# ouc-ocean-group/RRNet

Hardware: AMD Instinct MI355X
Metric: images/sec (train step) (higher is better)
Workload: dtype f32; 1 GPU; RRNet hourglass-104 (2 stacks) train step, 1024x1024 synthetic VisDrone frames, fp32; per_gpu_batch=8, global_batch=8, k=1500, parallelism=dp1

## Files before the change

rrnet_amd/_C.py:

```python
import ctypes
import os

import torch

_HERE = os.path.dirname(os.path.abspath(__file__))
LIB_PATH = os.path.join(_HERE, "librrnet_hip.so")
_lib = None

c_int, c_float, c_void_p, c_size_t = ctypes.c_int, ctypes.c_float, ctypes.c_void_p, ctypes.c_size_t
c_long, c_double = ctypes.c_long, ctypes.c_double


class RRNetHipError(RuntimeError):
    pass


def lib():
    global _lib
    if _lib is None:
        global LIB_PATH
        LIB_PATH = os.environ.get("RRNET_HIP_LIB", LIB_PATH)
        if not os.path.exists(LIB_PATH):
            raise RRNetHipError(
                "librrnet_hip.so not found at %s — build it with `python rrnet_amd/csrc/build.py` "
# ... 51 lines not shown
                    argtypes.append(_CTYPE[toks[0]])
                    pointees.append("hipStream_t" if toks[0] == "hipStream_t" else None)
        sigs[name] = Signature((restype, argtypes))
        sigs[name].pointees = tuple(pointees)
    return sigs


def header_signatures():
    global _SIGS
    if _SIGS is None:
        _SIGS = _parse_header(MAIN_HEADER)
    return _SIGS


MAIN_HEADER = "rrnet_hip.h"
COMPANION_HEADERS = ("rrnet_hip_se.h", "rrnet_hip_attn.h", "rrnet_hip_dw.h", "rrnet_hip_rows.h")
_FAMILY_SIGS = {}


def family_signatures(header):
    if header not in COMPANION_HEADERS:
        raise RRNetHipError("%s is not a header of this library (%s)" % (header, ", ".join((MAIN_HEADER,) + COMPANION_HEADERS)))
    if header not in _FAMILY_SIGS:
        _FAMILY_SIGS[header] = _parse_header(header)
    return _FAMILY_SIGS[header]


def declared(name):
    sig = header_signatures().get(name)
    if sig is not None:
        return sig, MAIN_HEADER
# ... 93 lines not shown
```

rrnet_amd/csrc/build.py:

```python
import os
import subprocess
import sys
from concurrent.futures import ThreadPoolExecutor

HERE = os.path.dirname(os.path.abspath(__file__))
ROOT = os.path.dirname(os.path.dirname(HERE))
INC = os.path.join(ROOT, "include")
OUT = os.path.join(os.path.dirname(HERE), "librrnet_hip.so")
HIPCC = os.environ.get("HIPCC", "/opt/rocm/bin/hipcc")
COMMON = ["--offload-arch=gfx950", "-O3", "-fPIC", "-std=c++17", "-I", INC, "-I", HERE,
          "-Wno-unused-result", "-fno-gpu-rdc"]
PER_FILE = {
    "softnms.hip": ["-ffp-contract=off"],
    "hardnms.hip": ["-ffp-contract=off"],
    "refine.hip": ["-ffp-contract=off"],
    "targets.hip": ["-ffp-contract=off"],
    "psroi.hip": ["-ffp-contract=off"],
    "augment.hip": ["-ffp-contract=off"],
    "augment_paste.hip": ["-ffp-contract=off"],
    "jitter.hip": ["-ffp-contract=off"],
    "evalmatch.hip": ["-ffp-contract=off"],
    "detect.hip": ["-ffp-contract=off"],
    "retina.hip": ["-ffp-contract=off"],
    "kmeans.hip": ["-ffp-contract=off"],
    "wbf.hip": ["-ffp-contract=off"],
    "textio.hip": ["-ffp-contract=off"],
    "depthwise.hip": ["-ffp-contract=off"],
}


def sources():
    return sorted(f for f in os.listdir(HERE) if f.endswith(".hip") or f.endswith(".cpp"))


def _stale(obj, src):
    if not os.path.exists(obj):
        return True
    t = os.path.getmtime(obj)
    deps = [os.path.join(HERE, src)] + [os.path.join(INC, h) for h in os.listdir(INC) if h.endswith(".h")] + \
           [os.path.join(HERE, h) for h in os.listdir(HERE) if h.endswith(".h")]
    return any(os.path.getmtime(d) > t for d in deps)

# ... 31 lines not shown
```

rrnet_amd/csrc/conv.hip:

```cpp
#include "conv_launch.h"
#include <hip/amd_detail/amd_hip_unsafe_atomics.h>

namespace {

typedef float f32x4 __attribute__((ext_vector_type(4)));
typedef float f32x16 __attribute__((ext_vector_type(16)));

__device__ float rr_zero16[4] = {0.f, 0.f, 0.f, 0.f};

constexpr int BM = 128;
constexpr int BK = 32;

struct ConvArgs {
    const float *src;
    const float *w;
    float *dst;
    const float *bias;
    double *stat_slab;
    const float *bs_y, *bs_z, *bs_mean, *bs_invstd, *bs_msc, *bs_msh;
    int bs_relu_bias;
    int N;
    int SH, SW, SC;
    int DH, DW, DC;
    int R, S, stride, pad_h, pad_w;
    int relu, accumulate;
    int M;
    int Kg;
    int wK, wC;
    const float *zero;
    int ksplit;
    int parity_order;
    int parity;
    int dst32;
    int pos_major;
    const int *gate;
    int gate_max;
};

__device__ __forceinline__ int xcd_remap(int bid, int nb)
{
    const int q = nb >> 3, r = nb & 7, xcd = bid & 7, idx = bid >> 3;
    return (xcd < r ? xcd * (q + 1) : r * (q + 1) + (xcd - r) * q) + idx;
}

template <int BN, int MODE, bool SCALAR, int BKT, int PIPE, bool BNS = false, bool POSM = false>
__global__ __launch_bounds__(256, PIPE == 2 ? 3 : 1) void conv_igemm_kernel(const ConvArgs a)
{
    static_assert(BKT == 32 && (PIPE == 0 || PIPE == 2), "conv_igemm_kernel: K-step 32, PIPE 0 or 2");
    if constexpr (MODE == 0 && !BNS && !POSM) {
        if (a.gate != nullptr && *a.gate <= a.gate_max) return;
    }
    constexpr int WN = BN / 64 ? BN / 64 : 1;
    constexpr int WM = 4 / WN;
    constexpr int TM = BM / (WM * 32);
    constexpr int TN = BN / (WN * 32);
    constexpr bool B_KN = (MODE == 1);
    constexpr int LDK = BKT + 4;
    constexpr int LDB = B_KN ? BN : LDK;
    constexpr int A_ELEMS = BM * LDK;
    constexpr int B_ELEMS = B_KN ? BKT * BN : BN * LDK;
    constexpr int CPR = BKT / 4;
    constexpr int RPP = 256 / CPR;
    constexpr int AJ = BM / RPP;
// ... 313 lines not shown
    auto sub = [&](const f32x4 (&fa)[TM], const f32x4 (&fb)[TN], int e) {
#pragma unroll
        for (int i = 0; i < TM; ++i)
#pragma unroll
            for (int j = 0; j < TN; ++j)
                acc[i][j] = __builtin_amdgcn_mfma_f32_32x32x2f32(fa[i][e], fb[j][e], acc[i][j], 0, 0, 0);
        __builtin_amdgcn_sched_barrier(0);
    };
    auto make_srd = [](const float *p, long bytes) {
        const unsigned long long u = reinterpret_cast<unsigned long long>(p);
        const unsigned lo = __builtin_amdgcn_readfirstlane((unsigned)u);
        const unsigned hi = __builtin_amdgcn_readfirstlane((unsigned)(u >> 32));
        void *q = reinterpret_cast<void *>(((unsigned long long)hi << 32) | lo);
        return __builtin_amdgcn_make_buffer_rsrc(q, 0, __builtin_amdgcn_readfirstlane((int)bytes), 0x00020000);
    };
    const __amdgpu_buffer_rsrc_t rs_src = make_srd(a.src, (long)a.N * a.SH * a.SW * a.SC * 4);
    const __amdgpu_buffer_rsrc_t rs_w = make_srd(a.w, (long)a.wK * RS * a.wC * 4);
    constexpr unsigned OOB = 0xFFFFFFF0u;
    int a_boff[AJ], b_boff[BJ];
#pragma unroll
    for (int j = 0; j < AJ; ++j) a_boff[j] = (int)(a_base[j] * 4);
#pragma unroll
    for (int j = 0; j < BJ; ++j) b_boff[j] = (int)(b_base[j] * 4);
    int p_cch = kc_lo / RSc, p_tl = kc_lo - (kc_lo / RSc) * RSc;
    int p_ri = p_tl / Sc, p_si = p_tl - (p_tl / Sc) * Sc;
    int p_adelta = 0, p_wdelta = 0, p_c0 = 0, p_tlc = 0;
    bool p_cok = false, p_wcok = false, p_live = true;
    auto prep = [&]() {
        const int tap = (r0 + tstep * p_ri) * a.S + (s0 + tstep * p_si);
        p_c0 = p_cch * BKT;
        p_tlc = p_tl;
        p_adelta = (sgn * (p_ri * a.SW + p_si) * a.SC + p_c0) * 4;
// ... 66 lines not shown
    }
    }

    double *sred = reinterpret_cast<double *>(lds);
    const bool do_stats = (MODE == 0) && a.stat_slab != nullptr && a.ksplit <= 1;
    constexpr bool bnsum = BNS;
    auto bs_srd = [](const float *p, long bytes) {
        const unsigned long long u = reinterpret_cast<unsigned long long>(p);
        const unsigned lo = __builtin_amdgcn_readfirstlane((unsigned)u);
        const unsigned hi = __builtin_amdgcn_readfirstlane((unsigned)(u >> 32));
        void *q = reinterpret_cast<void *>(((unsigned long long)hi << 32) | lo);
        return __builtin_amdgcn_make_buffer_rsrc(q, 0, __builtin_amdgcn_readfirstlane((int)bytes), 0x00020000);
    };
    const __amdgpu_buffer_rsrc_t bs_rs_y = bs_srd(BNS ? a.bs_y : a.src, (long)a.M * a.DC * 4);
    const __amdgpu_buffer_rsrc_t bs_rs_z = bs_srd(BNS && a.bs_z != nullptr ? a.bs_z : a.src, (long)a.M * a.DC * 4);
    const __amdgpu_buffer_rsrc_t rs_dst = bs_srd(a.dst, a.dst32 ? (long)a.M * a.DC * 4 : 0);
    constexpr unsigned OOBD = 0xFFFFFFF0u;
    const int mode_e = a.ksplit > 1 ? 2 : (a.accumulate ? 1 : 0);
    auto put_stats = [&](int j, float s1, float s2) {
        double d1 = (double)s1, d2 = (double)s2;
        d1 += __shfl_xor(d1, 32, 64);
        d2 += __shfl_xor(d2, 32, 64);
        if (lh == 0) {
            const int cl = (wn * TN + j) * 32 + lr;
            sred[(wm * BN + cl) * 2 + 0] = d1;
            sred[(wm * BN + cl) * 2 + 1] = d2;
        }
    };
    auto put_tile = [&](const f32x16 &c, const unsigned (&off)[16], float bv, float &s1, float &s2, int mode)
                        __attribute__((always_inline)) {
        const bool relu = MODE == 0 && a.relu;
// ... 620 lines not shown
    }
    if (bn == 64)
        return small ? IG(64, false, 2) : IG(64, false, 0);
    return scalar ? IG(32, true, 0) : IG(32, false, 0);
#undef IG
}

}

extern "C" size_t rr_conv_stat_slab_bytes(int n, int p, int q, int k)
{
    const long M = (long)n * p * q;
    return (size_t)((M + BM - 1) / BM) * 2 * k * sizeof(double);
}

int rr_conv_colstats(const float *y, long M, int C, double *slab, hipStream_t stream, const char *name)
{
    const int lanes = 256 / (C / 4);
    int sblocks = rr_cdiv(M, (long)lanes * 8);
    if (sblocks > 256) sblocks = 256;
    hipLaunchKernelGGL(colstats_kernel, dim3(sblocks), dim3(256), 0, stream, y, M, C, slab);
    RR_CHECK_LAUNCH(name);
    return RR_OK;
}

static int fprop_impl(const char *name, const float *x, const float *w, const float *bias, float *y, double *stat_slab,
                      int n, int h, int wd, int c, int k, int r, int s, int stride, int pad_h,
                      int pad_w, int relu, int accumulate, hipStream_t stream, const BnSumArgs *bs = nullptr, const int *gate = nullptr,
                      int gate_max = 0)
{
// ... 293 lines not shown
```

rrnet_amd/csrc/conv_launch.h:

```cpp
#pragma once
#include "common.h"
#include "conv_plan.h"
#include "rrnet_hip.h"
#include "rrnet_hip_rows.h"

struct BnSumArgs {
    const float *y, *z, *mean, *invstd, *msc, *msh;
    double *slab;
    double *sums;
    int relu_bias;
    bool bn_ok(int c) const { return y && mean && invstd && slab && sums && (!msc == !msh) && c % 4 == 0 && c <= 1024; }
    bool relu_bias_ok(int c, int k) const { return z && slab && sums && c % 4 == 0 && k % 4 == 0 && c <= 1024; }
    template <typename A> void into(A &a) const
    {
        a.stat_slab = slab; a.bs_y = y; a.bs_z = z; a.bs_mean = mean; a.bs_invstd = invstd; a.bs_msc = msc; a.bs_msh = msh; a.bs_relu_bias = relu_bias;
    }
};

template <typename K, typename A>
inline int rr_launch(K kern, dim3 grid, int threads, size_t lds, hipStream_t stream, const A &args, const char *name)
{
    if (lds > 48 * 1024)
        RR_CHECK_HIP(hipFuncSetAttribute(reinterpret_cast<const void *>(kern), hipFuncAttributeMaxDynamicSharedMemorySize, (int)lds), name);
    hipLaunchKernelGGL(kern, grid, dim3(threads), lds, stream, args);
    RR_CHECK_LAUNCH(name);
    return RR_OK;
}

inline int rr_refuse(const char *name, const rr_plan::Refusal &r)
{
    char why[256];
    snprintf(why, sizeof(why), r.why, r.a[0], r.a[1], r.a[2], r.a[3], r.a[4]);
    rr_set_error("%s: %s", name, why);
    return RR_ERR_ARG;
}

inline int rr_conv_link(const BnSumArgs *bs) { return bs == nullptr ? rr_plan::LINK_NONE : (bs->relu_bias ? rr_plan::LINK_RELU_BIAS : rr_plan::LINK_BN); }

int rr_conv_colstats(const float *y, long M, int C, double *slab, hipStream_t stream, const char *name);

int rr_gated_zero(float *p, size_t bytes, const int *count, int max_rows, int when_rows, hipStream_t stream, const char *name);

inline int rr_conv_before_launch(const rr_plan::FpropPlan &pl, int n, int k, float *y, double *stat_slab, hipStream_t stream, const char *name)
{
    RR_CHECK_HIP(rr_zero2(pl.zero_dst ? y : nullptr, pl.zero_dst ? sizeof(float) * (size_t)pl.M * k : 0, pl.zero_slab ? stat_slab : nullptr,
                          pl.zero_slab ? rr_conv_stat_slab_bytes(n, pl.dh, pl.dw, k) : 0, stream), name);
    return RR_OK;
}

inline int rr_conv_after_launch(const rr_plan::FpropPlan &pl, const BnSumArgs *bs, int k, const float *y, double *stat_slab, hipStream_t stream,
                                const char *name)
{
    switch (pl.after) {
    case rr_plan::AFTER_REDUCE_SLAB: return rr_bn_reduce_slab(bs->slab, rr_cdiv(pl.M, rr_plan::BM), k, bs->sums, stream);
// ... 64 lines not shown
```

rrnet_amd/csrc/conv_plan.h:

```cpp
#pragma once
#include <stdlib.h>

namespace rr_plan {

enum { MATH_F32 = 0, MATH_BF16 = 1, MATH_F16X3 = 2 };
enum { FAM_CONV16 = 3 };
enum { LINK_NONE = 0, LINK_BN = 1, LINK_RELU_BIAS = 2 };
enum { AFTER_NONE = 0, AFTER_REDUCE_SLAB = 1, AFTER_BWD_REDUCE = 2, AFTER_COLSTATS = 3 };

constexpr int BM = 128;
constexpr int BK = 32;

inline int cdiv(long a, long b) { return (int)((a + b - 1) / b); }

inline int mid_tiles() { return 48; }
inline int small_tiles() { return 16; }

inline int pick_ksplit(int blocks, int nk)
{
    static int enabled = -1;
    if (enabled < 0) {
        const char *e = getenv("RR_CONV_SPLITK");
        enabled = (e && atoi(e) == 0) ? 0 : 1;
    }
// ... 306 lines not shown

inline RowsPlan rows_plan(int max_rows, int c, int k, int r, int s)
{
    RowsPlan p{};
    p.dgrad_x = cdiv(max_rows, ROWS_DGRAD_BM);
    p.dgrad_y = cdiv(c, 128);
    p.mt = cdiv(k, 128); p.nt = cdiv(c, 128);
    const int tiles = p.mt * p.nt * r * s;
    p.splits = ROWS_WGRAD_SLOTS / tiles > 1 ? ROWS_WGRAD_SLOTS / tiles : 1;
    const int most = cdiv(cdiv(max_rows, BK), ROWS_WGRAD_MIN_CHUNKS);
    if (p.splits > most) p.splits = most;
    p.wgrad_grid = tiles * p.splits;
    return p;
}

}
```

rrnet_amd/flat.py:

```python
import os

import torch
import torch.distributed as dist

from rrnet_amd import dptrace, ops


class FlatParams:

    def __init__(self, module, bucket_elems=16 * 1024 * 1024):
        params = [p for p in module.parameters() if p.requires_grad]
        assert params, "no trainable parameters"
        dev = params[0].device
        offs, total = [], 0
        for p in params:
            offs.append(total)
            total += (p.numel() + 3) // 4 * 4
        self.flat = torch.zeros(total, dtype=torch.float32, device=dev)
        self.grad = torch.zeros(total, dtype=torch.float32, device=dev)
        self.params = params
        self.numel = total
        for p, o in zip(params, offs):
            n = p.numel()
            if p.dim() == 4:
# ... 17 lines not shown
            if end - start >= bucket_elems or i + 1 == len(params):
                self._bucket_range.append((start, end))
                self._bucket_need.append(need)
                start, need = end, 0
        self._index_of = {id(p): i for i, p in enumerate(params)}
        self._offs = {id(p): o for p, o in zip(params, offs)}
        self._names = {id(p): name for name, p in module.named_parameters()}
        self.wt_flat = None
        self.w16_flat = self.wt16_flat = None
        self._wt_table = None
        self._wt_tabled = set()
        self.epoch = 0
        self._wt_version = None
        self._wt_pver = {}
        self._wt_enabled = True and dev.type == "cuda"
        self.overlap = os.environ.get("RR_DP_OVERLAP", "1") != "0"
        self._pg = None
        self._begin_step()

    def _build_wt_table(self):
        import numpy as np
        rows = []
        self._wt_tabled = set()
        for p in self.params:
            if p.dim() != 4:
                continue
            k, c, r, s = p.shape
            if k > 65535 or r * s >= 2048 or (k + 31) // 32 > 1023 or (c + 31) // 32 > 1023:
                continue
            self._wt_tabled.add(id(p))
            o = self._offs[id(p)]
            kt, ct = (k + 31) // 32, (c + 31) // 32
            tap, ki, ci = np.meshgrid(np.arange(r * s), np.arange(kt), np.arange(ct), indexing="ij")
            n = tap.size
            t = np.empty((n, 4), dtype=np.int32)
            t[:, 0] = o
            t[:, 1] = ((r * s) << 16) | k
            t[:, 2] = c
            t[:, 3] = (tap.reshape(-1) << 20) | (ki.reshape(-1) << 10) | ci.reshape(-1)
            rows.append(t)
        tab = np.concatenate(rows) if rows else np.zeros((0, 4), dtype=np.int32)
        self._wt_table = torch.from_numpy(tab).to(self.flat.device)

    def refresh_wt(self):
        if not self._wt_enabled or self.wt_flat is None:
            return
        from rrnet_amd import _C
        if self.w16_flat is not None:
            _C.call("rr_weight_flip_transpose_batch_bf16", self.flat, self.wt_flat, self.w16_flat, self.wt16_flat, self._wt_table,
                    self._wt_table.shape[0])
        else:
            _C.call("rr_weight_flip_transpose_batch", self.flat, self.wt_flat, self._wt_table, self._wt_table.shape[0])
        self._wt_version = self.flat._version
        self._wt_pver = {id(p): p._version for p in self.params if p.dim() == 4}

    def invalidate_wt(self):
        self._wt_version = None
        self.epoch += 1

    def _wt_ready(self, p, bf16):
        if not self._wt_enabled or p.dim() != 4 or id(p) not in self._offs:
            return False
        if self.wt_flat is None:
            self._build_wt_table()
            self.wt_flat = torch.empty_like(self.flat)
            self._wt_version = None
        if bf16 and self.w16_flat is None:
            self.w16_flat = torch.empty(self.numel, dtype=torch.bfloat16, device=self.flat.device)
            self.wt16_flat = torch.empty(self.numel, dtype=torch.bfloat16, device=self.flat.device)
# ... 183 lines not shown
```

rrnet_amd/ops.py:

```python
import os
import sys
import threading
import types

import torch

from rrnet_amd import _C

CL = torch.channels_last


class KernelTimer:

    def __init__(self, only=None, every=1):
        self.records = []
        self.bytes = {}
        self.only = only
        self.every = max(int(every), 1)
        self.seen = {}

    def launch(self, name, flops, fn, detail=None, nbytes=0.0):
        if self.only is not None and name not in self.only:
            return fn()
        k = self.seen.get(name, 0)
# ... 415 lines not shown
        x16 = bf16_of(x)
        if w16 is None:
            w16 = bf16_of(w)
        if want_stats:
            slab = torch.empty(_C.call("rr_conv16_stat_slab_bytes", n, p, q, k) // 8, dtype=torch.float64, device=x.device)
        flops = 2.0 * n * p * q * k * (c * r * s if algo_kg is None else algo_kg)
        _launch("conv16_fprop", flops, "rr_conv16_fprop",
                (x16, w16, bias, None if y16 is not None else y, y16, slab, n, h, wd, c, k, r, s, stride, pad[0], pad[1], int(relu)),
                (n, h, wd, c, k, r, s, stride), 2.0 * (x.numel() + w.numel()) + (2.0 if y16 is not None else 4.0) * y.numel())
        return (y, slab) if want_stats else y
    if want_stats:
        nbytes = _C.call("rr_conv_stat_slab_bytes", n, p, q, k)
        slab = torch.empty(nbytes // 8, dtype=torch.float64, device=x.device)
    bf = _bf16_ok(c, 4 if _mode() != MATH_F16X3 else k, r, s, x, w, y, pixels=n * p * q)
    flops = 2.0 * n * p * q * k * (c * r * s if algo_kg is None else algo_kg)
    if bf == MATH_F16X3 and w_split is None:
        w_split = split_filter(w, amax_of(w), n * p * q)
    sfx, tag, tail = _math_call(bf, x, w, w16, w_split, takes_filter=True)
    _launch(_igemm_name("fprop", k, c % 4 != 0, n * p * q) + tag, flops, "rr_conv_fprop" + sfx,
            (x, w, bias, y, slab, n, h, wd, c, k, r, s, stride, pad[0], pad[1], int(relu)) + tail,
            (n, h, wd, c, k, r, s, stride), 4.0 * (x.numel() + y.numel() + w.numel()))
    return (y, slab) if want_stats else y


def conv_packable(x, w, stride):
    k, c, r, s = w.shape
    return c % 4 != 0 and 32 < r * s * c <= 512 and k >= 32 and not x.requires_grad


def conv_fprop_packed(x, w, stride, pad, want_stats=False):
# ... 178 lines not shown
            4.0 * (dy.numel() + out.numel() * ((2 if geo[9] else 1) + (link is not None)) + w.numel()))


def _dgrad_s2(dy, w, out, geo, flops, bf, conv16):
    src = bf16_of(dy) if conv16 else dy
    wsub = torch.empty(w.numel(), dtype=torch.bfloat16 if conv16 else torch.float32, device=dy.device)
    sfx, tag, tail = _math_call(bf, dy, w)
    _launch("conv16_dgrad_s2" if conv16 else "conv_dgrad_s2" + tag, flops, "rr_conv16_dgrad_s2" if conv16 else "rr_conv_dgrad_s2" + sfx,
            (src, w, out) + geo + (wsub,) + tail, geo[:7] + (2,))


def _dgrad_fp32(dy, w, out, geo, flops, stride):
    n, h, wd, c, k = geo[:5]
    _launch(_igemm_name("dgrad", c, (k % 4 != 0) or (c % 4 != 0), n * h * wd, stride), flops, "rr_conv_dgrad",
            (dy, w, out) + geo[:7] + (stride,) + geo[7:], geo[:7] + (stride,))


_ROWS = _C.Family("rrnet_hip_rows.h")
_CONV_ROWS = os.environ.get("RR_CONV_ROWS", "1") != "0"
_ROWS_MAX_SHARE = 8
_TARGETS_MAX_SHARE = 4


def active_rows(dy):
    m, k = dy.shape[0] * dy.shape[2] * dy.shape[3], dy.shape[1]
    rows = torch.empty(m, dtype=torch.int32, device=dy.device)
    count = torch.empty(1, dtype=torch.int32, device=dy.device)
    work = torch.empty(_ROWS.call("rr_active_rows_work_bytes", m) // 4, dtype=torch.int32, device=dy.device)
    _ROWS.call("rr_active_rows", dy, m, k, rows, count, work)
    return rows, count, work
# ... 36 lines not shown
        accumulate = False
    else:
        amax_drop(out)
    assert is_nhwc(out)
    link, link_b16, have_z = link_facts(bnsum, bnsum_z, x_shape)
    if link_b16 and link != "bn":
        bnsum_z = f32_of(bnsum_z)
    route, bf = dgrad_route(tuple(dy.shape), tuple(w.shape), x_shape, stride, pad, link, link_b16, have_z, dy.is_cuda)
    if is_phantom(dy) and route not in _DGRAD_DY16:
        dy = f32_of(dy)
    geo = (n, h, wd, c, k, r, s, pad[0], pad[1], int(accumulate))
    flops = 2.0 * dy.shape[0] * dy.shape[2] * dy.shape[3] * k * c * r * s
    listed = rows_side.now(dy) if route in ("fprop", "fprop_bnsum") and bf == MATH_F32 else None
    if listed is not None and _rows_shape_ok(dy, x_shape, w.shape, stride):
        _dgrad_rows_pair(dy, w, out, geo, wt, listed)
    elif route in ("conv16_s1", "relumask"):
        _dgrad_conv16_s1(dy, w, out, geo, flops, wt, wt16, *((bnsum, bnsum_z) if route == "relumask" else ()))
    elif route in ("relubias", "head"):
        _dgrad_relubias(dy, w, out, geo, flops, bf, bnsum, bnsum_z, wt, route == "head")
    elif route in ("fprop", "fprop_bnsum"):
        _dgrad_fprop(dy, w, out, geo, flops, bf, wt, wt16, wt_split, *((bnsum, bnsum_z) if route == "fprop_bnsum" else ()))
    elif route in ("conv16_s2", "parity_s2"):
        _dgrad_s2(dy, w, out, geo, flops, bf, route == "conv16_s2")
    else:
        _dgrad_fp32(dy, w, out, geo, flops, stride)
    return out


def conv_wgrad(x, dy, dw, stride=1, pad=(0, 0), explicit_out=False, algo_c=None):
    _C.require_cuda(x, dy, dw)
# ... 1620 lines not shown
```

Baseline: 18.84 images/sec.

## Add Winograd F(2x2,3x3) route for fp32 3x3 stride-1 conv fprop and dgrad

```diff
diff --git a/include/rrnet_hip_wino.h b/include/rrnet_hip_wino.h
--- /dev/null
+++ b/include/rrnet_hip_wino.h
@@ -0,0 +1,34 @@
+#ifndef RRNET_HIP_WINO_H
+#define RRNET_HIP_WINO_H
+
+#include <stddef.h>
+
+#ifdef __cplusplus
+extern "C" {
+#endif
+
+#ifndef __HIP_INCLUDE_HIP_HIP_RUNTIME_API_H__
+#ifndef RRNET_HIP_H
+typedef struct ihipStream_t *hipStream_t;
+#endif
+#endif
+
+#define RR_WINO_PLAN_INTS 11
+int rr_conv_wino_plan(int math, int n, int h, int wd, int c, int k, int r, int s, int stride, int pad_h, int pad_w, int out_h,
+                      int out_w, int flags, int *plan);
+size_t rr_conv_wino_ws_bytes(int n, int h, int wd, int c, int k);
+int rr_wino_filter(const float *w, float *u, int k, int c, hipStream_t stream);
+int rr_wino_filter_batch(const long long *table, int nfilters, hipStream_t stream);
+int rr_conv_wino_fprop(const float *x, const float *u, const float *bias, float *y, double *stat_slab, float *ws, size_t ws_bytes,
+                       int n, int h, int wd, int c, int k, int relu, int accumulate, hipStream_t stream);
+int rr_conv_wino_dgrad_bnsum(const float *dy, const float *u, float *dx, float *ws, size_t ws_bytes, int n, int h, int wd, int c,
+                             int k, int accumulate, const float *prod_y, const float *prod_z, const float *prod_mean,
+                             const float *prod_invstd, const float *prod_mask_scale, const float *prod_mask_shift, double *slab,
+                             double *sums, hipStream_t stream);
+int rr_wino_input(const float *x, float *v, int n, int h, int wd, int c, hipStream_t stream);
+int rr_wino_gemm(const float *v, const float *u, float *m, long tiles, int c, int k, hipStream_t stream);
+
+#ifdef __cplusplus
+}
+#endif
+#endif
diff --git a/rrnet_amd/_C.py b/rrnet_amd/_C.py
--- a/rrnet_amd/_C.py
+++ b/rrnet_amd/_C.py
@@ -89,7 +89,7 @@
 
 
 MAIN_HEADER = "rrnet_hip.h"
-COMPANION_HEADERS = ("rrnet_hip_se.h", "rrnet_hip_attn.h", "rrnet_hip_dw.h", "rrnet_hip_rows.h")
+COMPANION_HEADERS = ("rrnet_hip_se.h", "rrnet_hip_attn.h", "rrnet_hip_dw.h", "rrnet_hip_rows.h", "rrnet_hip_wino.h")
 _FAMILY_SIGS = {}
 
 
diff --git a/rrnet_amd/csrc/build.py b/rrnet_amd/csrc/build.py
--- a/rrnet_amd/csrc/build.py
+++ b/rrnet_amd/csrc/build.py
@@ -26,6 +26,7 @@
     "wbf.hip": ["-ffp-contract=off"],
     "textio.hip": ["-ffp-contract=off"],
     "depthwise.hip": ["-ffp-contract=off"],
+    "conv_wino.hip": ["-ffp-contract=off"],
 }
 
 
diff --git a/rrnet_amd/csrc/conv.hip b/rrnet_amd/csrc/conv.hip
--- a/rrnet_amd/csrc/conv.hip
+++ b/rrnet_amd/csrc/conv.hip
@@ -35,6 +35,7 @@
     int pos_major;
     const int *gate;
     int gate_max;
+    long batch_src, batch_w, batch_dst;
 };
 
 __device__ __forceinline__ int xcd_remap(int bid, int nb)
@@ -43,10 +44,11 @@
     return (xcd < r ? xcd * (q + 1) : r * (q + 1) + (xcd - r) * q) + idx;
 }
 
-template <int BN, int MODE, bool SCALAR, int BKT, int PIPE, bool BNS = false, bool POSM = false>
+template <int BN, int MODE, bool SCALAR, int BKT, int PIPE, bool BNS = false, bool POSM = false, bool BATCH = false>
 __global__ __launch_bounds__(256, PIPE == 2 ? 3 : 1) void conv_igemm_kernel(const ConvArgs a)
 {
     static_assert(BKT == 32 && (PIPE == 0 || PIPE == 2), "conv_igemm_kernel: K-step 32, PIPE 0 or 2");
+    static_assert(!BATCH || (MODE == 0 && PIPE == 2 && !BNS && !POSM), "conv_igemm_kernel: BATCH is for the pipelined plain forward kernel");
     if constexpr (MODE == 0 && !BNS && !POSM) {
         if (a.gate != nullptr && *a.gate <= a.gate_max) return;
     }
@@ -390,8 +392,8 @@
         void *q = reinterpret_cast<void *>(((unsigned long long)hi << 32) | lo);
         return __builtin_amdgcn_make_buffer_rsrc(q, 0, __builtin_amdgcn_readfirstlane((int)bytes), 0x00020000);
     };
-    const __amdgpu_buffer_rsrc_t rs_src = make_srd(a.src, (long)a.N * a.SH * a.SW * a.SC * 4);
-    const __amdgpu_buffer_rsrc_t rs_w = make_srd(a.w, (long)a.wK * RS * a.wC * 4);
+    const __amdgpu_buffer_rsrc_t rs_src = make_srd(BATCH ? a.src + (long)blockIdx.y * a.batch_src : a.src, (long)a.N * a.SH * a.SW * a.SC * 4);
+    const __amdgpu_buffer_rsrc_t rs_w = make_srd(BATCH ? a.w + (long)blockIdx.y * a.batch_w : a.w, (long)a.wK * RS * a.wC * 4);
     constexpr unsigned OOB = 0xFFFFFFF0u;
     int a_boff[AJ], b_boff[BJ];
 #pragma unroll
@@ -488,7 +490,7 @@
     };
     const __amdgpu_buffer_rsrc_t bs_rs_y = bs_srd(BNS ? a.bs_y : a.src, (long)a.M * a.DC * 4);
     const __amdgpu_buffer_rsrc_t bs_rs_z = bs_srd(BNS && a.bs_z != nullptr ? a.bs_z : a.src, (long)a.M * a.DC * 4);
-    const __amdgpu_buffer_rsrc_t rs_dst = bs_srd(a.dst, a.dst32 ? (long)a.M * a.DC * 4 : 0);
+    const __amdgpu_buffer_rsrc_t rs_dst = bs_srd(BATCH ? a.dst + (long)blockIdx.y * a.batch_dst : a.dst, a.dst32 ? (long)a.M * a.DC * 4 : 0);
     constexpr unsigned OOBD = 0xFFFFFFF0u;
     const int mode_e = a.ksplit > 1 ? 2 : (a.accumulate ? 1 : 0);
     auto put_stats = [&](int j, float s1, float s2) {
@@ -1139,6 +1141,24 @@
     return (size_t)((M + BM - 1) / BM) * 2 * k * sizeof(double);
 }
 
+int rr_conv_wino_gemm(const float *v, const float *u, float *m, long tiles, int c, int k, hipStream_t stream, const char *name)
+{
+    RR_CHECK_ARG(tiles > 0 && c > 0 && k > 0 && c % 4 == 0 && k % 4 == 0 && tiles * c * 4 < (1l << 31) && tiles * k * 4 < (1l << 31)
+                 && (long)k * c * 4 < (1l << 31), "%s: bad GEMM geometry", name);
+    ConvArgs a{};
+    a.src = v; a.w = u; a.dst = m; a.zero = zero_page();
+    a.N = 1; a.SH = 1; a.SW = (int)tiles; a.SC = c;
+    a.DH = 1; a.DW = (int)tiles; a.DC = k;
+    a.R = 1; a.S = 1; a.stride = 1; a.ksplit = 1;
+    a.M = (int)tiles; a.Kg = c; a.wK = k; a.wC = c; a.dst32 = 1;
+    a.batch_src = tiles * c; a.batch_w = (long)k * c; a.batch_dst = tiles * k;
+    const int bn = k > 64 ? 128 : 64;
+    const dim3 grid(rr_cdiv(tiles, BM) * rr_cdiv(k, bn), 16, 1);
+    if (bn == 128)
+        return rr_launch(conv_igemm_kernel<128, 0, false, BK, 2, false, false, true>, grid, 256, igemm_lds(128, false, 1), stream, a, name);
+    return rr_launch(conv_igemm_kernel<64, 0, false, BK, 2, false, false, true>, grid, 256, igemm_lds(64, false, 1), stream, a, name);
+}
+
 int rr_conv_colstats(const float *y, long M, int C, double *slab, hipStream_t stream, const char *name)
 {
     const int lanes = 256 / (C / 4);
diff --git a/rrnet_amd/csrc/conv_launch.h b/rrnet_amd/csrc/conv_launch.h
--- a/rrnet_amd/csrc/conv_launch.h
+++ b/rrnet_amd/csrc/conv_launch.h
@@ -38,6 +38,8 @@
 inline int rr_conv_link(const BnSumArgs *bs) { return bs == nullptr ? rr_plan::LINK_NONE : (bs->relu_bias ? rr_plan::LINK_RELU_BIAS : rr_plan::LINK_BN); }
 
 int rr_conv_colstats(const float *y, long M, int C, double *slab, hipStream_t stream, const char *name);
+
+int rr_conv_wino_gemm(const float *v, const float *u, float *m, long tiles, int c, int k, hipStream_t stream, const char *name);
 
 int rr_gated_zero(float *p, size_t bytes, const int *count, int max_rows, int when_rows, hipStream_t stream, const char *name);
 
diff --git a/rrnet_amd/csrc/conv_plan.h b/rrnet_amd/csrc/conv_plan.h
--- a/rrnet_amd/csrc/conv_plan.h
+++ b/rrnet_amd/csrc/conv_plan.h
@@ -344,4 +344,47 @@
     return p;
 }
 
-}
+constexpr long WINO_MIN_PIXELS = 65536;
+constexpr int WINO_OUT_LANES = 4;
+struct WinoPlan {
+    const char *refuse;
+    int floor_only;
+    int th, tw;
+    long tiles;
+    int bn;
+    int gemm_blocks;
+    int out_x, out_y;
+    int tiles_per_wg;
+    long ws_bytes;
+};
+
+inline WinoPlan wino_plan(int math, const ConvGeom &g, const ConvFlags &f)
+{
+    WinoPlan p{};
+    const long G2 = 1l << 31;
+#define RR_PLAN_REFUSE(cond, why) do { if (cond) { p.refuse = why; return p; } } while (0)
+    RR_PLAN_REFUSE(!(g.n > 0 && g.h > 0 && g.w > 0 && g.c > 0 && g.k > 0), "bad dims");
+    RR_PLAN_REFUSE(math != MATH_F32, "fp32 arithmetic only");
+    RR_PLAN_REFUSE(!(g.r == 3 && g.s == 3 && g.stride == 1 && g.pad_h == 1 && g.pad_w == 1), "3x3, stride 1, pad 1 only");
+    RR_PLAN_REFUSE(g.out_h > 0 || g.out_w > 0, "no explicit output size");
+    RR_PLAN_REFUSE(!(g.c % 4 == 0 && g.k % 4 == 0), "C and K must be multiples of 4");
+    RR_PLAN_REFUSE(f.strided_dst, "no strided destination");
+    RR_PLAN_REFUSE(f.link == LINK_RELU_BIAS, "the conv + bias + ReLU link is not built on this route");
+    RR_PLAN_REFUSE(f.link == LINK_BN && (f.bias || f.relu || f.stats || g.k > 1024), "a BatchNorm link: plain data gradient, at most 1024 channels");
+    const long M = (long)g.n * g.h * g.w;
+    p.th = (g.h + 1) / 2; p.tw = (g.w + 1) / 2;
+    p.tiles = (long)g.n * p.th * p.tw;
+    RR_PLAN_REFUSE(!(M * g.c * 4 < G2 && M * g.k * 4 < G2 && 9l * g.c * g.k * 4 < G2 && p.tiles * g.c * 4 < G2 && p.tiles * g.k * 4 < G2),
+                   "tensors must stay below 2 GiB");
+    p.bn = g.k > 64 ? 128 : 64;
+    p.gemm_blocks = cdiv(p.tiles, BM) * cdiv(g.k, p.bn);
+    p.out_x = cdiv(M, BM);
+    p.out_y = cdiv(g.k / 4, 64);
+    p.tiles_per_wg = cdiv(p.tiles, p.out_x);
+    p.ws_bytes = 16l * p.tiles * ((long)g.c + g.k) * 4;
+    if (M < WINO_MIN_PIXELS) { p.refuse = "fewer output pixels than the route's floor"; p.floor_only = 1; }
+#undef RR_PLAN_REFUSE
+    return p;
+}
+
+}
diff --git a/rrnet_amd/csrc/conv_wino.hip b/rrnet_amd/csrc/conv_wino.hip
--- /dev/null
+++ b/rrnet_amd/csrc/conv_wino.hip
@@ -0,0 +1,360 @@
+#include "conv_launch.h"
+#include "rrnet_hip_wino.h"
+
+namespace {
+
+typedef float f32x4 __attribute__((ext_vector_type(4)));
+
+__device__ __forceinline__ __amdgpu_buffer_rsrc_t wino_srd(const void *p, long bytes)
+{
+    const unsigned long long u = reinterpret_cast<unsigned long long>(p);
+    const unsigned lo = __builtin_amdgcn_readfirstlane((unsigned)u);
+    const unsigned hi = __builtin_amdgcn_readfirstlane((unsigned)(u >> 32));
+    void *q = reinterpret_cast<void *>(((unsigned long long)hi << 32) | lo);
+    return __builtin_amdgcn_make_buffer_rsrc(q, 0, __builtin_amdgcn_readfirstlane((int)bytes), 0x00020000);
+}
+constexpr unsigned OOB = 0xFFFFFFF0u;
+__device__ __forceinline__ f32x4 wino_load(__amdgpu_buffer_rsrc_t rs, unsigned off)
+{
+    return __builtin_bit_cast(f32x4, __builtin_amdgcn_raw_buffer_load_b128(rs, off, 0, 0));
+}
+
+struct WinoFilterRow { const float *w; float *u; long K, C; };
+
+__global__ __launch_bounds__(256) void wino_filter_kernel(const WinoFilterRow *table, const WinoFilterRow one)
+{
+    const WinoFilterRow d = table != nullptr ? table[blockIdx.y] : one;
+    const long KC = d.K * d.C;
+    for (long idx = (long)blockIdx.x * 256 + threadIdx.x; idx < KC; idx += (long)gridDim.x * 256) {
+        const long ko = idx / d.C, c = idx - ko * d.C;
+        float g[3][3], t[4][3];
+#pragma unroll
+        for (int r = 0; r < 3; ++r)
+#pragma unroll
+            for (int s = 0; s < 3; ++s) g[r][s] = d.w[(ko * 9 + r * 3 + s) * d.C + c];
+#pragma unroll
+        for (int s = 0; s < 3; ++s) {
+            t[0][s] = g[0][s];
+            t[1][s] = 0.5f * ((g[0][s] + g[2][s]) + g[1][s]);
+            t[2][s] = 0.5f * ((g[0][s] + g[2][s]) - g[1][s]);
+            t[3][s] = g[2][s];
+        }
+#pragma unroll
+        for (int a = 0; a < 4; ++a) {
+            const float u0 = t[a][0], u3 = t[a][2];
+            const float u1 = 0.5f * ((t[a][0] + t[a][2]) + t[a][1]);
+            const float u2 = 0.5f * ((t[a][0] + t[a][2]) - t[a][1]);
+            d.u[(4 * a + 0) * KC + idx] = u0;
+            d.u[(4 * a + 1) * KC + idx] = u1;
+            d.u[(4 * a + 2) * KC + idx] = u2;
+            d.u[(4 * a + 3) * KC + idx] = u3;
+        }
+    }
+}
+
+__global__ __launch_bounds__(256) void wino_input_kernel(const float *x, float *v, int H, int W, int C, int TH, int TW, long tiles,
+                                                         long x_bytes)
+{
+    const __amdgpu_buffer_rsrc_t rs = wino_srd(x, x_bytes);
+    const int C4 = C / 4;
+    const long total = tiles * C4;
+    for (long idx = (long)blockIdx.x * 256 + threadIdx.x; idx < total; idx += (long)gridDim.x * 256) {
+        const long t = idx / C4;
+        const int c = (int)(idx - t * C4) * 4;
+        const int tw = (int)(t % TW);
+        const long rest = t / TW;
+        const int th = (int)(rest % TH);
+        const int n = (int)(rest / TH);
+        const int h0 = 2 * th - 1, w0 = 2 * tw - 1;
+        f32x4 d[4][4];
+#pragma unroll
+        for (int i = 0; i < 4; ++i)
+#pragma unroll
+            for (int j = 0; j < 4; ++j) {
+                const int ih = h0 + i, iw = w0 + j;
+                const bool in = (unsigned)ih < (unsigned)H && (unsigned)iw < (unsigned)W;
+                const unsigned off = in ? (unsigned)((((n * H + ih) * W + iw) * C + c) * 4) : OOB;
+                d[i][j] = wino_load(rs, off);
+            }
+        f32x4 m[4][4];
+#pragma unroll
+        for (int j = 0; j < 4; ++j) {
+            m[0][j] = d[0][j] - d[2][j];
+            m[1][j] = d[1][j] + d[2][j];
+            m[2][j] = d[2][j] - d[1][j];
+            m[3][j] = d[1][j] - d[3][j];
+        }
+        float *vp = v + t * C + c;
+        const long bs = tiles * C;
+#pragma unroll
+        for (int a = 0; a < 4; ++a) {
+            *reinterpret_cast<f32x4 *>(vp + (4 * a + 0) * bs) = m[a][0] - m[a][2];
+            *reinterpret_cast<f32x4 *>(vp + (4 * a + 1) * bs) = m[a][1] + m[a][2];
+            *reinterpret_cast<f32x4 *>(vp + (4 * a + 2) * bs) = m[a][2] - m[a][1];
+            *reinterpret_cast<f32x4 *>(vp + (4 * a + 3) * bs) = m[a][1] - m[a][3];
+        }
+    }
+}
+
+struct WinoOutArgs {
+    const float *m;
+    float *y;
+    const float *bias;
+    double *slab;
+    const float *bs_y, *bs_z, *bs_mean, *bs_invstd, *bs_msc, *bs_msh;
+    int H, W, K, TH, TW;
+    long tiles, y_bytes;
+    int per_wg, relu, accumulate;
+};
+
+template <bool LINK>
+__global__ __launch_bounds__(256) void wino_output_kernel(const WinoOutArgs a)
+{
+    __shared__ double sred[rr_plan::WINO_OUT_LANES][64][8];
+    const int t = threadIdx.x, cl = t & 63, tl = t >> 6;
+    const int c = (blockIdx.y * 64 + cl) * 4;
+    const bool c_ok = c < a.K;
+    const int cm = c_ok ? c : 0;
+    const __amdgpu_buffer_rsrc_t rs_y = wino_srd(a.y, a.y_bytes);
+    const __amdgpu_buffer_rsrc_t rs_py = wino_srd(LINK ? a.bs_y : a.y, a.y_bytes);
+    const __amdgpu_buffer_rsrc_t rs_pz = wino_srd(LINK && a.bs_z != nullptr ? a.bs_z : a.y, a.y_bytes);
+    const bool use_z = LINK && a.bs_z != nullptr;
+    const f32x4 zero4 = {0.f, 0.f, 0.f, 0.f};
+    f32x4 bv = zero4, bs_m = zero4, bs_i = zero4, bs_sc = zero4, bs_sh = zero4;
+    if (c_ok) {
+        if (a.bias != nullptr) bv = *reinterpret_cast<const f32x4 *>(a.bias + c);
+        if constexpr (LINK) {
+            bs_m = *reinterpret_cast<const f32x4 *>(a.bs_mean + c);
+            bs_i = *reinterpret_cast<const f32x4 *>(a.bs_invstd + c);
+            if (a.bs_z == nullptr) {
+                if (a.bs_msc != nullptr) {
+                    bs_sc = *reinterpret_cast<const f32x4 *>(a.bs_msc + c);
+                    bs_sh = *reinterpret_cast<const f32x4 *>(a.bs_msh + c);
+                } else {
+                    bs_sh = f32x4{1.f, 1.f, 1.f, 1.f};
+                }
+            }
+        }
+    }
+    const bool want_sums = a.slab != nullptr;
+    double d1[4] = {0, 0, 0, 0}, d2[4] = {0, 0, 0, 0};
+    f32x4 s1 = zero4, s2 = zero4;
+    int chain = 0;
+    const long t_lo = (long)blockIdx.x * a.per_wg;
+    const long t_hi = t_lo + a.per_wg < a.tiles ? t_lo + a.per_wg : a.tiles;
+    const long mb = a.tiles * a.K;
+    for (long tile = t_lo + tl; tile < t_hi; tile += rr_plan::WINO_OUT_LANES) {
+        const int tw = (int)(tile % a.TW);
+        const long rest = tile / a.TW;
+        const int th = (int)(rest % a.TH);
+        const int n = (int)(rest / a.TH);
+        const float *mp = a.m + tile * a.K + cm;
+        f32x4 m[4][4];
+#pragma unroll
+        for (int i = 0; i < 16; ++i) m[i >> 2][i & 3] = *reinterpret_cast<const f32x4 *>(mp + i * mb);
+        unsigned off[2][2];
+#pragma unroll
+        for (int r = 0; r < 2; ++r)
+#pragma unroll
+            for (int q = 0; q < 2; ++q) {
+                const int oh = 2 * th + r, ow = 2 * tw + q;
+                off[r][q] = (c_ok && oh < a.H && ow < a.W) ? (unsigned)((((n * a.H + oh) * a.W + ow) * a.K + c) * 4) : OOB;
+            }
+        f32x4 old[2][2], py[2][2], pz[2][2];
+#pragma unroll
+        for (int r = 0; r < 2; ++r)
+#pragma unroll
+            for (int q = 0; q < 2; ++q) {
+                old[r][q] = a.accumulate ? wino_load(rs_y, off[r][q]) : zero4;
+                if constexpr (LINK) {
+                    py[r][q] = wino_load(rs_py, off[r][q]);
+                    pz[r][q] = use_z ? wino_load(rs_pz, off[r][q]) : zero4;
+                }
+            }
+        f32x4 w[2][4];
+#pragma unroll
+        for (int j = 0; j < 4; ++j) {
+            w[0][j] = (m[0][j] + m[1][j]) + m[2][j];
+            w[1][j] = (m[1][j] - m[2][j]) - m[3][j];
+        }
+#pragma unroll
+        for (int r = 0; r < 2; ++r) {
+            f32x4 o[2];
+            o[0] = (w[r][0] + w[r][1]) + w[r][2];
+            o[1] = (w[r][1] - w[r][2]) - w[r][3];
+#pragma unroll
+            for (int q = 0; q < 2; ++q) {
+                f32x4 v = o[q] + bv;
+                if (a.relu) {
+#pragma unroll
+                    for (int e = 0; e < 4; ++e) v[e] = v[e] > 0.f ? v[e] : 0.f;
+                }
+                if (a.accumulate) v += old[r][q];
+                __builtin_amdgcn_raw_buffer_store_b128(__builtin_bit_cast(__attribute__((ext_vector_type(4))) unsigned, v), rs_y, off[r][q], 0, 0);
+                const bool live = off[r][q] != OOB;
+                if constexpr (LINK) {
+                    const f32x4 aff = rr_bn_affine4(py[r][q], bs_sc, bs_sh);
+#pragma unroll
+                    for (int e = 0; e < 4; ++e) {
+                        const bool on = use_z ? pz[r][q][e] > 0.f : aff[e] > 0.f;
+                        const float dd = (on && live) ? v[e] : 0.f;
+                        s1[e] += dd;
+                        s2[e] += dd * ((py[r][q][e] - bs_m[e]) * bs_i[e]);
+                    }
+                } else {
+#pragma unroll
+                    for (int e = 0; e < 4; ++e) {
+                        const float vm = live ? v[e] : 0.f;
+                        s1[e] += vm;
+                        s2[e] += vm * vm;
+                    }
+                }
+            }
+        }
+        if (++chain == 8) {
+#pragma unroll
+            for (int e = 0; e < 4; ++e) { d1[e] += (double)s1[e]; d2[e] += (double)s2[e]; }
+            s1 = zero4; s2 = zero4; chain = 0;
+        }
+    }
+    if (!want_sums) return;
+#pragma unroll
+    for (int e = 0; e < 4; ++e) {
+        sred[tl][cl][e] = d1[e] + (double)s1[e];
+        sred[tl][cl][4 + e] = d2[e] + (double)s2[e];
+    }
+    __syncthreads();
+    if (tl == 0 && c_ok) {
+        double *row = a.slab + (long)blockIdx.x * 2 * a.K;
+#pragma unroll
+        for (int e = 0; e < 4; ++e) {
+            double r1 = 0.0, r2 = 0.0;
+#pragma unroll
+            for (int l = 0; l < rr_plan::WINO_OUT_LANES; ++l) { r1 += sred[l][cl][e]; r2 += sred[l][cl][4 + e]; }
+            row[c + e] = r1;
+            row[a.K + c + e] = r2;
+        }
+    }
+}
+
+int grid_for(long threads)
+{
+    long blocks = (threads + 255) / 256;
+    return (int)(blocks > 256 * 64 ? 256 * 64 : (blocks < 1 ? 1 : blocks));
+}
+
+int run_filter(const WinoFilterRow *table, const WinoFilterRow &one, int nfilters, int blocks_x, hipStream_t stream, const char *name)
+{
+    hipLaunchKernelGGL(wino_filter_kernel, dim3(blocks_x, nfilters), dim3(256), 0, stream, table, one);
+    RR_CHECK_LAUNCH(name);
+    return RR_OK;
+}
+
+int run_input(const float *x, float *v, int n, int h, int wd, int c, const rr_plan::WinoPlan &pl, hipStream_t stream, const char *name)
+{
+    hipLaunchKernelGGL(wino_input_kernel, dim3(grid_for(pl.tiles * (c / 4))), dim3(256), 0, stream, x, v, h, wd, c, pl.th, pl.tw, pl.tiles,
+                       (long)n * h * wd * c * 4);
+    RR_CHECK_LAUNCH(name);
+    return RR_OK;
+}
+
+int checked_plan(const char *name, int n, int h, int wd, int c, int k, const rr_plan::ConvFlags &f, size_t ws_bytes, rr_plan::WinoPlan *pl)
+{
+    *pl = rr_plan::wino_plan(rr_plan::MATH_F32, {n, h, wd, c, k, 3, 3, 1, 1, 1, 0, 0}, f);
+    RR_CHECK_ARG(pl->refuse == nullptr || pl->floor_only, "%s: %s", name, pl->refuse);
+    RR_CHECK_ARG(ws_bytes >= (size_t)pl->ws_bytes, "%s: workspace of %ld bytes needed (rr_conv_wino_ws_bytes)", name, pl->ws_bytes);
+    return RR_OK;
+}
+
+int run_route(const char *name, const float *x, const float *u, float *y, float *ws, int n, int h, int wd, int c, int k,
+              const rr_plan::WinoPlan &pl, WinoOutArgs &o, bool link, hipStream_t stream)
+{
+    float *v = ws, *m = ws + 16 * pl.tiles * c;
+    if (int rc = run_input(x, v, n, h, wd, c, pl, stream, name)) return rc;
+    if (int rc = rr_conv_wino_gemm(v, u, m, pl.tiles, c, k, stream, name)) return rc;
+    o.m = m; o.y = y; o.y_bytes = (long)n * h * wd * k * 4; o.H = h; o.W = wd; o.K = k; o.TH = pl.th; o.TW = pl.tw; o.tiles = pl.tiles; o.per_wg = pl.tiles_per_wg;
+    if (link) hipLaunchKernelGGL(wino_output_kernel<true>, dim3(pl.out_x, pl.out_y), dim3(256), 0, stream, o);
+    else hipLaunchKernelGGL(wino_output_kernel<false>, dim3(pl.out_x, pl.out_y), dim3(256), 0, stream, o);
+    RR_CHECK_LAUNCH(name);
+    return RR_OK;
+}
+
+}
+
+extern "C" int rr_conv_wino_plan(int math, int n, int h, int wd, int c, int k, int r, int s, int stride, int pad_h, int pad_w, int out_h,
+                                 int out_w, int flags, int *plan)
+{
+    RR_CHECK_ARG(plan != nullptr && ((flags >> 8) & 3) <= rr_plan::LINK_RELU_BIAS, "rr_conv_wino_plan: bad arguments");
+    const rr_plan::WinoPlan pl = rr_plan::wino_plan(math, {n, h, wd, c, k, r, s, stride, pad_h, pad_w, out_h, out_w},
+                                                    {(flags & 1) != 0, (flags & 2) != 0, (flags & 4) != 0, (flags >> 8) & 3, (flags & 8) != 0,
+                                                     (flags & 16) != 0});
+    const int out[RR_WINO_PLAN_INTS] = {pl.refuse == nullptr, pl.floor_only, (int)(pl.tiles & 0x7fffffff), (int)(pl.tiles >> 31), pl.bn, pl.gemm_blocks, pl.out_x,
+                                        pl.out_y, pl.tiles_per_wg, (int)(pl.ws_bytes & 0x7fffffff), (int)(pl.ws_bytes >> 31)};
+    for (int i = 0; i < RR_WINO_PLAN_INTS; ++i) plan[i] = out[i];
+    return RR_OK;
+}
+
+extern "C" size_t rr_conv_wino_ws_bytes(int n, int h, int wd, int c, int k)
+{
+    if (n <= 0 || h <= 0 || wd <= 0 || c <= 0 || k <= 0) return 0;
+    return (size_t)16 * n * ((h + 1) / 2) * ((wd + 1) / 2) * ((size_t)c + k) * sizeof(float);
+}
+
+extern "C" int rr_wino_filter_batch(const long long *table, int nfilters, hipStream_t stream)
+{
+    static_assert(sizeof(WinoFilterRow) == 4 * sizeof(long long), "rr_wino_filter_batch: four 64-bit words per filter");
+    RR_CHECK_ARG(table != nullptr && nfilters >= 0 && nfilters < 65536, "rr_wino_filter_batch: bad arguments");
+    if (nfilters == 0) return RR_OK;
+    return run_filter(reinterpret_cast<const WinoFilterRow *>(table), WinoFilterRow{}, nfilters, 64, stream, "rr_wino_filter_batch");
+}
+
+extern "C" int rr_wino_filter(const float *w, float *u, int k, int c, hipStream_t stream)
+{
+    RR_CHECK_ARG(w != nullptr && u != nullptr && k > 0 && c > 0, "rr_wino_filter: bad arguments");
+    return run_filter(nullptr, WinoFilterRow{w, u, k, c}, 1, grid_for((long)k * c), stream, "rr_wino_filter");
+}
+
+extern "C" int rr_wino_input(const float *x, float *v, int n, int h, int wd, int c, hipStream_t stream)
+{
+    rr_plan::WinoPlan pl;
+    if (int rc = checked_plan("rr_wino_input", n, h, wd, c, c, {}, (size_t)-1, &pl)) return rc;
+    RR_CHECK_ARG(x != nullptr && v != nullptr, "rr_wino_input: null argument");
+    return run_input(x, v, n, h, wd, c, pl, stream, "rr_wino_input");
+}
+
+extern "C" int rr_wino_gemm(const float *v, const float *u, float *m, long tiles, int c, int k, hipStream_t stream)
+{
+    RR_CHECK_ARG(v != nullptr && u != nullptr && m != nullptr, "rr_wino_gemm: null argument");
+    return rr_conv_wino_gemm(v, u, m, tiles, c, k, stream, "rr_wino_gemm");
+}
+
+extern "C" int rr_conv_wino_fprop(const float *x, const float *u, const float *bias, float *y, double *stat_slab, float *ws, size_t ws_bytes,
+                                  int n, int h, int wd, int c, int k, int relu, int accumulate, hipStream_t stream)
+{
+    rr_plan::WinoPlan pl;
+    if (int rc = checked_plan("rr_conv_wino_fprop", n, h, wd, c, k,
+                              {bias != nullptr, relu != 0, stat_slab != nullptr, rr_plan::LINK_NONE, accumulate != 0, false}, ws_bytes, &pl))
+        return rc;
+    RR_CHECK_ARG(x != nullptr && u != nullptr && y != nullptr && ws != nullptr, "rr_conv_wino_fprop: null argument");
+    WinoOutArgs o{};
+    o.bias = bias; o.slab = stat_slab; o.relu = relu != 0; o.accumulate = accumulate != 0;
+    return run_route("rr_conv_wino_fprop", x, u, y, ws, n, h, wd, c, k, pl, o, false, stream);
+}
+
+extern "C" int rr_conv_wino_dgrad_bnsum(const float *dy, const float *u, float *dx, float *ws, size_t ws_bytes, int n, int h, int wd, int c,
+                                        int k, int accumulate, const float *prod_y, const float *prod_z, const float *prod_mean,
+                                        const float *prod_invstd, const float *prod_mask_scale, const float *prod_mask_shift, double *slab,
+                                        double *sums, hipStream_t stream)
+{
+    const char *name = "rr_conv_wino_dgrad_bnsum";
+    const BnSumArgs bs{prod_y, prod_z, prod_mean, prod_invstd, prod_mask_scale, prod_mask_shift, slab, sums, 0};
+    RR_CHECK_ARG(bs.bn_ok(c) && dy != nullptr && u != nullptr && dx != nullptr && ws != nullptr,
+                 "%s: bad arguments (every tensor, the producer's tensors and the two buffers; C %% 4 == 0, C <= 1024)", name);
+    rr_plan::WinoPlan pl;
+    if (int rc = checked_plan(name, n, h, wd, k, c, {false, false, false, rr_plan::LINK_BN, accumulate != 0, false}, ws_bytes, &pl)) return rc;
+    WinoOutArgs o{};
+    o.slab = slab; o.accumulate = accumulate != 0;
+    o.bs_y = prod_y; o.bs_z = prod_z; o.bs_mean = prod_mean; o.bs_invstd = prod_invstd; o.bs_msc = prod_mask_scale; o.bs_msh = prod_mask_shift;
+    if (int rc = run_route(name, dy, u, dx, ws, n, h, wd, k, c, pl, o, true, stream)) return rc;
+    return rr_bn_reduce_slab(slab, pl.out_x, c, sums, stream);
+}
diff --git a/rrnet_amd/flat.py b/rrnet_amd/flat.py
--- a/rrnet_amd/flat.py
+++ b/rrnet_amd/flat.py
@@ -55,6 +55,11 @@
         self._wt_version = None
         self._wt_pver = {}
         self._wt_enabled = True and dev.type == "cuda"
+        self._p_at = {o: p for p, o in zip(params, offs) if p.dim() == 4}
+        self._wino, self._wino_rows, self._wino_table = {}, [], None
+        self._wino_version, self._wino_pver = None, {}
+        if self._wt_enabled:
+            ops.FLAT_BUFFERS.add(self)
         self.overlap = os.environ.get("RR_DP_OVERLAP", "1") != "0"
         self._pg = None
         self._begin_step()
@@ -84,16 +89,47 @@
         self._wt_table = torch.from_numpy(tab).to(self.flat.device)
 
     def refresh_wt(self):
-        if not self._wt_enabled or self.wt_flat is None:
+        if not self._wt_enabled:
             return
         from rrnet_amd import _C
-        if self.w16_flat is not None:
-            _C.call("rr_weight_flip_transpose_batch_bf16", self.flat, self.wt_flat, self.w16_flat, self.wt16_flat, self._wt_table,
-                    self._wt_table.shape[0])
-        else:
-            _C.call("rr_weight_flip_transpose_batch", self.flat, self.wt_flat, self._wt_table, self._wt_table.shape[0])
-        self._wt_version = self.flat._version
-        self._wt_pver = {id(p): p._version for p in self.params if p.dim() == 4}
+        if self.wt_flat is not None:
+            if self.w16_flat is not None:
+                _C.call("rr_weight_flip_transpose_batch_bf16", self.flat, self.wt_flat, self.w16_flat, self.wt16_flat, self._wt_table,
+                        self._wt_table.shape[0])
+            else:
+                _C.call("rr_weight_flip_transpose_batch", self.flat, self.wt_flat, self._wt_table, self._wt_table.shape[0])
+            self._wt_version = self.flat._version
+            self._wt_pver = {id(p): p._version for p in self.params if p.dim() == 4}
+        self._refresh_wino()
+
+    def _refresh_wino(self):
+        if not self._wino:
+            return
+        if self._wino_table is None:
+            self._wino_table = torch.tensor(self._wino_rows, dtype=torch.int64, device=self.flat.device)
+        ops._WINO.call("rr_wino_filter_batch", self._wino_table, len(self._wino_rows))
+        self._wino_version = (self.flat._version, self.epoch)
+        self._wino_pver = {id(p): p._version for p in self._p_at.values()}
+
+    def wino_view(self, w, flipped):
+        if not self._wt_enabled or w.device != self.flat.device:
+            return None
+        off = w.data_ptr() - self.flat.data_ptr()
+        p = self._p_at.get(off // 4) if 0 <= off < self.numel * 4 and off % 4 == 0 else None
+        if p is None or tuple(w.shape) != tuple(p.shape) or w.stride() != p.stride():
+            return None
+        if flipped and self.wt_view(p) is None:
+            return None
+        u = self._wino.get((off, flipped))
+        if u is None:
+            k, c = p.shape[:2]
+            u = self._wino[(off, flipped)] = torch.empty(16 * k * c, dtype=torch.float32, device=self.flat.device)
+            src = self.wt_flat if flipped else self.flat
+            self._wino_rows.append([src.data_ptr() + off, u.data_ptr(), c if flipped else k, k if flipped else c])
+            self._wino_table = self._wino_version = None
+        if self._wino_version != (self.flat._version, self.epoch) or self._wino_pver.get(id(p)) != p._version:
+            self._refresh_wino()
+        return u
 
     def invalidate_wt(self):
         self._wt_version = None
diff --git a/rrnet_amd/ops.py b/rrnet_amd/ops.py
--- a/rrnet_amd/ops.py
+++ b/rrnet_amd/ops.py
@@ -2,6 +2,7 @@
 import sys
 import threading
 import types
+import weakref
 
 import torch
 
@@ -453,6 +454,12 @@
         slab = torch.empty(nbytes // 8, dtype=torch.float64, device=x.device)
     bf = _bf16_ok(c, 4 if _mode() != MATH_F16X3 else k, r, s, x, w, y, pixels=n * p * q)
     flops = 2.0 * n * p * q * k * (c * r * s if algo_kg is None else algo_kg)
+    if bf == MATH_F32 and wino_takes(n, h, wd, c, k, r, s, stride, pad, bias is not None, relu, want_stats):
+        u, ws = _wino_filter(w, False), _wino_ws(x.device, n, h, wd, c, k)
+        _launch("conv_fprop<wino>", flops * 16.0 / 36.0, "rr_conv_wino_fprop",
+                (x, u, bias, y, slab, ws, ws.numel() * 4, n, h, wd, c, k, int(relu), 0), (n, h, wd, c, k, r, s, stride),
+                4.0 * (x.numel() + y.numel() + w.numel()) + 2.0 * ws.numel() * 4.0, call=_WINO.call)
+        return (y, slab) if want_stats else y
     if bf == MATH_F16X3 and w_split is None:
         w_split = split_filter(w, amax_of(w), n * p * q)
     sfx, tag, tail = _math_call(bf, x, w, w16, w_split, takes_filter=True)
@@ -661,6 +668,68 @@
     n, h, wd, c, k = geo[:5]
     _launch(_igemm_name("dgrad", c, (k % 4 != 0) or (c % 4 != 0), n * h * wd, stride), flops, "rr_conv_dgrad",
             (dy, w, out) + geo[:7] + (stride,) + geo[7:], geo[:7] + (stride,))
+
+
+_WINO = _C.Family("rrnet_hip_wino.h")
+_CONV_WINO = os.environ.get("RR_CONV_WINO", "1") != "0"
+_WINO_BELOW_FLOOR = False
+_WINO_TAKES = {}
+_WINO_PLAN_FN = []
+_WINO_WS = {}
+FLAT_BUFFERS = weakref.WeakSet()
+
+
+def wino_takes(n, h, wd, c, k, r, s, stride, pad, bias=False, relu=False, stats=False, accumulate=False, link=False):
+    if not _CONV_WINO:
+        return False
+    key = (n, h, wd, c, k, r, s, stride, pad[0], pad[1], int(bias) | int(relu) << 1 | int(stats) << 2 | int(accumulate) << 3 | int(link) << 8)
+    hit = _WINO_TAKES.get(key)
+    if hit is None:
+        if not _WINO_PLAN_FN:
+            f, (sig, _) = getattr(_C.lib(), "rr_conv_wino_plan"), _C.declared("rr_conv_wino_plan")
+            f.restype, f.argtypes = sig[0], sig[1]
+            _WINO_PLAN_FN.append(f)
+        plan = (_C.c_int * 11)()
+        _C.check(_WINO_PLAN_FN[0](MATH_F32, *key[:10], 0, 0, key[10], plan), "rr_conv_wino_plan")
+        hit = _WINO_TAKES[key] = (bool(plan[0]), bool(plan[1]))
+    return hit[0] or (hit[1] and _WINO_BELOW_FLOOR)
+
+
+def _wino_ws(device, n, h, wd, c, k):
+    need = _WINO.call("rr_conv_wino_ws_bytes", n, h, wd, c, k) // 4
+    key = (device, torch.cuda.current_stream(device).cuda_stream)
+    ws = _WINO_WS.get(key)
+    if ws is None or ws.numel() < need:
+        _WINO_WS[key] = None
+        ws = _WINO_WS[key] = torch.empty(need, dtype=torch.float32, device=device)
+    return ws
+
+
+def _wino_filter(w, flipped, wt=None):
+    for flat in FLAT_BUFFERS:
+        u = flat.wino_view(w, flipped)
+        if u is not None:
+            return u
+    k, c = w.shape[0], w.shape[1]
+    src = _flipped_filter(w, wt, None, False)[0] if flipped else w
+    u = torch.empty(16 * k * c, dtype=torch.float32, device=w.device)
+    _WINO.call("rr_wino_filter", src, u, *((c, k) if flipped else (k, c)))
+    return u
+
+
+def _dgrad_wino(dy, w, out, geo, flops, wt, link=None, z=None):
+    n, h, wd, c, k = geo[:5]
+    u, ws = _wino_filter(w, True, wt), _wino_ws(dy.device, n, h, wd, k, c)
+    nbytes = 4.0 * (dy.numel() + out.numel() * ((2 if geo[9] else 1) + (link is not None)) + w.numel()) + 2.0 * ws.numel() * 4.0
+    if link is None:
+        _launch("conv_dgrad<wino>", flops * 16.0 / 36.0, "rr_conv_wino_fprop",
+                (dy, u, None, out, None, ws, ws.numel() * 4, n, h, wd, k, c, 0, geo[9]), geo[:7] + (1,), nbytes, call=_WINO.call)
+        return
+    slab = torch.empty(_C.call("rr_conv_stat_slab_bytes", n, h, wd, c) // 8, dtype=torch.float64, device=dy.device)
+    link.sums, link.dz = _ZEROS.take(2 * c, dy.device), out
+    _launch("conv_dgrad<wino>+bnsum", flops * 16.0 / 36.0, "rr_conv_wino_dgrad_bnsum",
+            (dy, u, out, ws, ws.numel() * 4, n, h, wd, c, k, geo[9], link.y, z if link.use_z else None, link.mean, link.invstd, link.msc,
+             link.msh, slab, link.sums), geo[:7] + (1,), nbytes, call=_WINO.call)
 
 
 _ROWS = _C.Family("rrnet_hip_rows.h")
@@ -727,6 +796,9 @@
     listed = rows_side.now(dy) if route in ("fprop", "fprop_bnsum") and bf == MATH_F32 else None
     if listed is not None and _rows_shape_ok(dy, x_shape, w.shape, stride):
         _dgrad_rows_pair(dy, w, out, geo, wt, listed)
+    elif (route in ("fprop", "fprop_bnsum") and bf == MATH_F32
+          and wino_takes(n, h, wd, k, c, r, s, stride, (r - 1 - pad[0], s - 1 - pad[1]), accumulate=accumulate, link=route == "fprop_bnsum")):
+        _dgrad_wino(dy, w, out, geo, flops, wt, *((bnsum, bnsum_z) if route == "fprop_bnsum" else ()))
     elif route in ("conv16_s1", "relumask"):
         _dgrad_conv16_s1(dy, w, out, geo, flops, wt, wt16, *((bnsum, bnsum_z) if route == "relumask" else ()))
     elif route in ("relubias", "head"):
```

After: 21.26 images/sec (median of 6 runs). +12.8%, better.
